# jedisct1/zig-lz4

Hardware: AMD Instinct MI355X
Metric: GiB/s uncompressed, block compress+decompress (higher is better)
Workload: dtype u8

## Files before the change

### zig-lz4_amd/csrc/zlz4_decompress.hip

```cpp
#include <cstdlib>
#include <type_traits>

#include "zlz4_device.hpp"
#include "zlz4_launch.hpp"

#ifdef ZLZ4_STAMPS
__device__ unsigned long long g_zlz4_dstamps[16];
#define DSTAMP_DECL unsigned long long st_acc[16] = {0,0,0,0,0,0,0,0,0,0,0,0,0,0,0,0}; unsigned long long st_last = __builtin_amdgcn_s_memtime();
#define DSTAMP(i) do { unsigned long long st_now; __builtin_amdgcn_sched_barrier(0); \
                      asm volatile("s_memtime %0\n\ts_waitcnt lgkmcnt(0)" : "=s"(st_now) :: "memory"); \
                      __builtin_amdgcn_sched_barrier(0); st_acc[i] += st_now - st_last; st_last = st_now; } while (0)
#define DSTAMP_ADD(i, n) do { st_acc[i] += (n); } while (0)
#define DSTAMP_FLUSH do { if (lane == 0) for (int st_k = 0; st_k < 16; st_k++) atomicAdd(&g_zlz4_dstamps[st_k], st_acc[st_k]); } while (0)
#else
#define DSTAMP_DECL
#define DSTAMP(i)
#define DSTAMP_ADD(i, n)
#define DSTAMP_FLUSH
#endif

namespace zlz4 {

__device__ __forceinline__ uint32_t ld16(const uint8_t *p) { uint16_t v; __builtin_memcpy(&v, p, 2); return v; }
__device__ __forceinline__ uint64_t ld64u(const uint8_t *p) { uint64_t v; __builtin_memcpy(&v, p, 8); return v; }

template <bool kWrite, bool kLaneCopy = false, bool kPhases = kLaneCopy, bool kDict = false, bool kBound = false,
          bool kPartial = false>
__global__ __launch_bounds__(256) __attribute__((amdgpu_waves_per_eu(kDict ? 8 : 1))) void k_decompress_safe(
    const uint8_t *__restrict__ d_in, const uint64_t *__restrict__ d_in_off,
    const uint32_t *__restrict__ d_in_len, uint8_t *d_out, const uint64_t *__restrict__ d_out_off,
    const uint32_t *__restrict__ d_out_cap, int64_t *__restrict__ d_result, uint32_t nblocks, uint32_t min_phase_tokens,
    const uint8_t *__restrict__ d_dict, const uint64_t *__restrict__ d_dict_off, const uint32_t *__restrict__ d_dict_len) {
    constexpr uint32_t short_max = kLaneCopy ? 32u : 0u;
    const uint32_t lane = threadIdx.x & 63u;
    const uint32_t blk = rfl(blockIdx.x * (blockDim.x >> 6) + (threadIdx.x >> 6));
    if (blk >= nblocks) return;

    const uint8_t *src = d_in + d_in_off[blk];
    uint8_t *dst = d_out + d_out_off[blk];
    const uint32_t iend = rfl(d_in_len[blk]);
    const uint32_t oend = rfl(d_out_cap[blk]);
    uint32_t lo = 0;
    if constexpr (kBound) {
        lo = rfl(d_dict_len[nblocks + blk]);
        if (lo >= kBoundInvalid) {
            if (lane == 0 && lo == kBoundInvalid) d_result[blk] = kErrInvalidState;
            return;
        }
    }
    const uint8_t *dend = nullptr, *dbase = nullptr;
    uint32_t dlen = 0;
    if constexpr (kDict) {
        const uint32_t dl = rfl(d_dict_len[blk]);
        dend = d_dict + d_dict_off[blk] + dl;
        dbase = dend - 65536;
        dlen = dl < 65536u ? dl : 65536u;
    }

    int64_t res = 0;
    uint32_t ip = 0, op = 0;

    if (iend != 0 && oend != 0) {
        uint32_t wbase = 0;
        uint32_t w = (lane < iend) ? src[lane] : 0u;
        DSTAMP_DECL
        uint32_t pml = 0, po = 0, pof = 0;
        u32x4 pa = {0, 0, 0, 0}, pb = {0, 0, 0, 0};
        constexpr uint32_t kNone = 0xFFFFFFFFu;
        uint32_t pd0 = 0, pd1 = 0, pdo0 = kNone, pdo1 = kNone;
        auto flush_pending = [&]() {
            if (!kWrite) return;
            if constexpr (kLaneCopy) {
                if (pdo0 != kNone) __builtin_memcpy(dst + pdo0, &pd0, 4);
                if (pdo1 != kNone) __builtin_memcpy(dst + pdo1, &pd1, 4);
                pdo0 = pdo1 = kNone;
            }
            if (pml != 0) {
                if (pml >= 16u) {
                    st128(dst + po, pa);
                    for (uint32_t k = 80u; k + 16u <= pml; k += 16u)
                        st128(dst + (po + k), ld128(kDict && po < pof ? dend - (pof - po) + k : dst + (po - pof + k)));
                    st128(dst + (po + pml - 16u), pb);
                } else if (pml >= 8u) {
                    const uint32_t sh = pml - 8u;
                    const bool hi4 = sh >= 4u;
                    const uint32_t x = hi4 ? pa.y : pa.x, y = hi4 ? pa.z : pa.y, z = hi4 ? pa.w : pa.z;
                    const u32x2 a = {pa.x, pa.y};
                    const u32x2 b = {__builtin_amdgcn_alignbyte(y, x, sh & 3u), __builtin_amdgcn_alignbyte(z, y, sh & 3u)};
                    __builtin_memcpy(dst + po, &a, 8); __builtin_memcpy(dst + (po + sh), &b, 8);
                } else {
                    const uint32_t sh = pml - 4u;
                    const uint32_t a = pa.x, b = __builtin_amdgcn_alignbyte(pa.y, pa.x, sh);
                    __builtin_memcpy(dst + po, &a, 4); __builtin_memcpy(dst + (po + sh), &b, 4);
                }
            }
            pml = 0;
        };
        auto reload = [&](uint32_t pos) {
            wbase = pos;
            w = (pos + lane < iend) ? src[pos + lane] : 0u;
        };
        auto fetch = [&](uint32_t pos) -> uint32_t {
            if (pos - wbase >= 64u) reload(pos);
            return rdlane(w, pos - wbase);
        };

        for (;;) {
            if (ip >= iend) break;
            if constexpr (kPartial) { if (op >= oend) break; }
            DSTAMP(6);
            if ((uint64_t)ip + 68u <= iend) {
              auto woff = [&](uint32_t p) { const uint32_t a = p + lane; return a + 4u <= iend ? a : iend - 4u; };
              auto wload_async = [&](uint32_t p) {
                  uint32_t r;
                  asm volatile("global_load_dword %0, %1, %2" : "=v"(r) : "v"(woff(p)), "s"(src) : "memory");
                  return r;
              };
              uint32_t xbase = ip, tdummy = 0;
              uint32_t X0 = ld32(src + woff(xbase)), X1 = ld32(src + woff(xbase + 64u));
              uint32_t X2 = wload_async(xbase + 128u);
              asm volatile("s_waitcnt vmcnt(0)" : "+v"(X2), "+v"(X0), "+v"(X1));
              for (;;) {
                const uint32_t xi = ip - xbase + lane;
                const uint32_t xa = shfl(X0, xi & 63u), xb = shfl(X1, xi & 63u);
                const uint32_t w4 = xi < 64u ? xa : xb;
                const uint32_t b0 = w4 & 0xFFu, b1 = (w4 >> 8) & 0xFFu;
                uint32_t lit = b0 >> 4, hl = 1u;
                bool cx = false;
                if (lit == 15u) { cx = (b1 == 255u); lit += b1; hl = 2u; }
                const uint32_t mpos = lane + hl + lit;
                const uint32_t mw = shfl(w4, mpos & 63u);
                const uint32_t off = mw & 0xFFFFu;
                uint32_t mlc = b0 & 15u, slen = hl + lit + 2u;
                if (mlc == 15u) { const uint32_t e2 = (mw >> 16) & 0xFFu; cx = cx || (e2 == 255u); mlc += e2; slen += 1u; }
                const uint32_t ml = mlc + kMinMatch;
                const uint32_t nxt = lane + slen;
                const bool ok = !cx && mpos <= 63u && nxt <= 64u && off != 0u;
                const uint32_t ol = lit + ml;
                const uint32_t pkv = ok ? (nxt | (ol << 7)) : 0xFFFFFFFFu;
                DSTAMP(0);
                const uint32_t orem = oend - op;
                const uint32_t room0 = kWrite ? (orem >= 32u ? orem - 32u : 0u) : orem;
                const uint32_t room = rfl(room0 < 4095u ? room0 : 4095u);
                uint32_t pos, T, wa, wpk, wt;
                uint64_t R;
                const uint64_t okm = ballot(ok);
                const uint32_t pk2v = nxt | ((nxt < 64u && ((okm >> (nxt & 63u)) & 1ull)) ? 0x80u : 0u) | (ol << 8);
                if (room0 >= 7100u && (okm & 1ull)) {
                    asm volatile(
                        "s_mov_b64 %[R], 0\n\t"
                        "s_mov_b32 %[T], 0\n\t"
                        "s_mov_b32 %[A], 0\n\t"
                        "s_nop 3\n"
                        "1:\n\t"
                        "v_readlane_b32 %[pk], %[pkv], %[A]\n\t"
                        "s_and_b32 %[B], %[pk], 0x7f\n\t"
                        "s_bitset1_b64 %[R], %[A]\n\t"
                        "s_lshr_b32 %[t], %[pk], 8\n\t"
                        "s_add_u32 %[T], %[T], %[t]\n\t"
                        "s_bitcmp1_b32 %[pk], 7\n\t"
                        "s_cbranch_scc0 4f\n\t"
                        "v_readlane_b32 %[pk], %[pkv], %[B]\n\t"
                        "s_and_b32 %[A], %[pk], 0x7f\n\t"
                        "s_bitset1_b64 %[R], %[B]\n\t"
                        "s_lshr_b32 %[t], %[pk], 8\n\t"
                        "s_add_u32 %[T], %[T], %[t]\n\t"
                        "s_bitcmp1_b32 %[pk], 7\n\t"
                        "s_cbranch_scc1 1b\n\t"
                        "s_mov_b32 %[B], %[A]\n"
                        "4:\n"
                        : [R] "=&s"(R), [T] "=&s"(T), [A] "=&s"(wa), [B] "=&s"(pos), [pk] "=&s"(wpk), [t] "=&s"(wt)
                        : [pkv] "v"(pk2v)
                        : "scc");
                } else
                asm volatile(
                    "s_mov_b64 %[R], 0\n\t"
                    "s_mov_b32 %[T], 0\n\t"
                    "s_mov_b32 %[A], 0\n\t"
                    "s_nop 3\n"
                    "1:\n\t"
                    "v_readlane_b32 %[pk], %[pkv], %[A]\n\t"
                    "s_and_b32 %[B], %[pk], 0x7f\n\t"
                    "s_lshr_b32 %[t], %[pk], 7\n\t"
                    "s_add_u32 %[t], %[t], %[T]\n\t"
                    "s_cmp_gt_u32 %[t], %[room]\n\t"
                    "s_cbranch_scc1 3f\n\t"
                    "s_bitset1_b64 %[R], %[A]\n\t"
                    "s_mov_b32 %[T], %[t]\n\t"
                    "s_cmp_gt_u32 %[B], 63\n\t"
                    "s_cbranch_scc1 4f\n\t"
                    "v_readlane_b32 %[pk], %[pkv], %[B]\n\t"
                    "s_and_b32 %[A], %[pk], 0x7f\n\t"
                    "s_lshr_b32 %[t], %[pk], 7\n\t"
                    "s_add_u32 %[t], %[t], %[T]\n\t"
                    "s_cmp_gt_u32 %[t], %[room]\n\t"
                    "s_cbranch_scc1 4f\n\t"
                    "s_bitset1_b64 %[R], %[B]\n\t"
                    "s_mov_b32 %[T], %[t]\n\t"
                    "s_cmp_lt_u32 %[A], 64\n\t"
                    "s_cbranch_scc1 1b\n"
                    "3:\n\t"
                    "s_mov_b32 %[B], %[A]\n"
                    "4:\n"
                    : [R] "=&s"(R), [T] "=&s"(T), [A] "=&s"(wa), [B] "=&s"(pos), [pk] "=&s"(wpk), [t] "=&s"(wt)
                    : [pkv] "v"(pkv), [room] "s"(room)
                    : "scc");
                DSTAMP(1);
                uint32_t relv = 0;
                const uint64_t R_walk = R;
                const uint32_t T_walk = T, pos_walk = pos;
                bool viol_err = false;
                const uint32_t op0 = op;
                if (R != 0) {
                    const bool real0 = in_mask(R);
                    const uint32_t x = real0 ? ol : 0u;
                    relv = wave_incl_scan(x) - x;
                    const uint32_t lit0 = rdlane(lit, 0);
                    viol_err = off + lo > op0 + relv + lit;
                    if constexpr (kDict) {
                        const uint32_t pr = op0 + relv + lit, need = kLaneCopy ? ml : (ml > 16u ? ml : 16u);
                        viol_err = viol_err && (off - pr < need || off - pr > dlen);
                    }
                    bool viol = viol_err;
                    if (kWrite) viol = viol || (off + lit0 < relv + ol);
                    const uint64_t vm = R & ballot(viol);
                    if (vm != 0) {
                        const uint32_t fb = first_lane(vm);
                        R &= (1ull << fb) - 1ull;
                        T = rdlane(relv, fb);
                        pos = fb;
                    }
                }
                DSTAMP(2);
                asm volatile("s_waitcnt vmcnt(1)" : "+v"(X2), "+v"(pa), "+v"(pb), "+v"(pd0), "+v"(pd1), "+v"(tdummy));
                if (R == 0) break;
                DSTAMP_ADD(8, 1);
                auto cap_short = [&]() {
                    if constexpr (kWrite && kLaneCopy) {
                        if ((uint32_t)__popcll(R) <= 16u) return;
                        const uint64_t S = R & ballot(ml <= short_max);
                        if ((uint32_t)__popcll(S) > 16u) {
                            const uint32_t fb = first_lane(S & ballot(lane_rank(S) == 16u));
                            R &= (1ull << fb) - 1ull;
                            T = rdlane(relv, fb);
                            pos = fb;
                            DSTAMP_ADD(13, 1);
                        }
                    }
                };
                auto copy_side = [&](auto later_phase) {
                if (kWrite) {
                    flush_pending();
                    DSTAMP(7);
                    const uint64_t below = R & (~0ull >> (63u - lane));
                    const uint32_t kl = 63u - (uint32_t)__builtin_clzll(below | 1ull);
                    const uint32_t q = shfl(relv | (lit << 16), kl);
                    const uint32_t qlit = q >> 16;
                    const uint32_t d = lane - kl - (qlit >= 15u ? 2u : 1u);
                    if (d < qlit && (!decltype(later_phase)::value || below != 0)) dst[op0 + (q & 0xFFFFu) + d] = (uint8_t)b0;
                    DSTAMP(3);
                    const uint64_t Sm = R & ballot(ml <= short_max), Lm = R & ~Sm;
                    const uint32_t po_t = op0 + relv + lit;
                    [[maybe_unused]] const bool shortm = in_mask(Sm);
                    const uint64_t H1 = (Lm & ballot(ml > 32u)) << 1, H2 = (Lm & ballot(ml > 64u)) << 2;
                    const uint32_t om = off | (ml << 16);
                    const uint32_t om1 = wave_shr1(om), po1 = wave_shr1(po_t);
                    const uint32_t om2 = wave_shr1(om1), po2 = wave_shr1(po1);
                    if (in_mask(Lm | H1 | H2)) {
                        const bool h1 = in_mask(H1), h2 = in_mask(H2);
                        const uint32_t t_om = h1 ? om1 : (h2 ? om2 : om), t_po = h1 ? po1 : (h2 ? po2 : po_t);
                        const uint32_t t_off = t_om & 0xFFFFu, t_ml = t_om >> 16;
                        const uint32_t pf = h1 ? 16u : (h2 ? 48u : 0u);
                        const uint32_t rest = t_ml - 16u - pf;
                        const uint32_t pl = pf == 0u ? t_ml : (rest < 16u ? 16u : (rest < 32u ? rest : 32u));
                        static_assert(!kLaneCopy || short_max >= 15u, "a lane-copy token lane must hold >= 16 bytes");
                        if constexpr (kDict) {
                            const uint64_t ma = (t_off > t_po ? (uint64_t)(uintptr_t)dbase + (t_po - t_off + 65536u)
                                                              : (uint64_t)(uintptr_t)dst + (t_po - t_off)) + pf;
                            asm volatile("global_load_dwordx4 %0, %1, off" : "+v"(pa) : "v"(ma) : "memory");
                            if (kLaneCopy || pl >= 16u)
                                asm volatile("global_load_dwordx4 %0, %1, off" : "+v"(pb) : "v"(ma + (pl - 16u)) : "memory");
                        } else {
                            const uint32_t mo = t_po - t_off + pf;
                            asm volatile("global_load_dwordx4 %0, %1, %2" : "+v"(pa) : "v"(mo), "s"(dst) : "memory");
                            if (kLaneCopy || pl >= 16u)
                                asm volatile("global_load_dwordx4 %0, %1, %2" : "+v"(pb) : "v"(mo + pl - 16u), "s"(dst) : "memory");
                        }
                        pml = pl; po = t_po + pf; pof = t_off;
                    }
                    if constexpr (kLaneCopy) {
                        const uint32_t ns = (uint32_t)__popcll(Sm);
                        const uint32_t rk = lane_rank(Sm);
                        const uint32_t lead = (lane & ~7u) << 2, k4 = (lane & 7u) * 4u, grp = lane >> 3;
                        auto round = [&](uint32_t g0, uint32_t &pd, uint32_t &pdo) {
                            const uint32_t rel = rk - g0;
                            const uint32_t dest = (shortm && rel < 8u ? rel * 8u : 63u) << 2;
                            const uint32_t s_po = (uint32_t)__builtin_amdgcn_ds_permute((int)dest, (int)po_t);
                            const uint32_t s_om = (uint32_t)__builtin_amdgcn_ds_permute((int)dest, (int)(off | (ml << 16)));
                            const uint32_t g_po = (uint32_t)__builtin_amdgcn_ds_bpermute((int)lead, (int)s_po);
                            const uint32_t g_om = (uint32_t)__builtin_amdgcn_ds_bpermute((int)lead, (int)s_om);
                            const uint32_t g_ml = g_om >> 16, g_mo = g_po - (g_om & 0xFFFFu);
                            const bool act = g0 + grp < ns && k4 < g_ml;
                            const uint32_t pk = k4 + 4u <= g_ml ? k4 : g_ml - 4u;
                            if (act) {
                                if constexpr (kDict) {
                                    const uint64_t ga = g_po < (g_om & 0xFFFFu) ? (uint64_t)(uintptr_t)dbase + (g_mo + pk + 65536u)
                                                                                : (uint64_t)(uintptr_t)dst + (g_mo + pk);
                                    asm volatile("global_load_dword %0, %1, off" : "+v"(pd) : "v"(ga) : "memory");
                                } else
                                    asm volatile("global_load_dword %0, %1, %2" : "+v"(pd) : "v"(g_mo + pk), "s"(dst) : "memory");
                                pdo = g_po + pk;
                            }
                        };
                        round(0u, pd0, pdo0);
                        if (ns > 8u) round(8u, pd1, pdo1);
                    }
                    DSTAMP(4);
                }
                };
                cap_short();
                DSTAMP_ADD(9, __builtin_popcountll(R));
                copy_side(std::false_type{});
                if constexpr (kWrite && kPhases) {
                    for (uint32_t phase = 1; phase < 6u && pos != pos_walk; phase++) {
                        const uint32_t first = pos, tbase = T;
                        const uint64_t Rn = R_walk & ~((1ull << first) - 1ull);
                        if ((uint32_t)__builtin_popcountll(Rn) < min_phase_tokens) break;
                        const uint32_t lit_f = rdlane(lit, first);
                        const bool violn = viol_err || (off + lit_f < (relv - tbase) + ol);
                        const uint64_t vmn = Rn & ballot(violn);
                        if ((vmn >> first) & 1ull) break;
                        if (vmn != 0) {
                            const uint32_t fb = first_lane(vmn);
                            R = Rn & ((1ull << fb) - 1ull);
                            T = rdlane(relv, fb);
                            pos = fb;
                        } else {
                            R = Rn; T = T_walk; pos = pos_walk;
                        }
                        DSTAMP_ADD(12, 1);
                        cap_short();
                        DSTAMP_ADD(9, __builtin_popcountll(R));
                        asm volatile("s_waitcnt vmcnt(0)" : "+v"(pa), "+v"(pb), "+v"(pd0), "+v"(pd1), "+v"(tdummy), "+v"(X2));
                        copy_side(std::true_type{});
#ifdef ZLZ4_STAMPS
                        if (phase == 5u && pos != pos_walk) DSTAMP_ADD(14, 1);
#endif
                    }
                }
                op += T;
                ip += pos;
                if ((uint64_t)ip + 68u > iend) break;
                {
                    const bool adv = ip - xbase >= 64u;
                    X0 = adv ? X1 : X0; X1 = adv ? X2 : X1; xbase += adv ? 64u : 0u;
                    X2 = wload_async(xbase + 128u);
                    const uint32_t ta = xbase + 128u + 1024u;
                    const uint32_t toff = ta < iend ? ta : iend - 1u;
                    asm volatile("global_load_ubyte %0, %1, %2" : "+v"(tdummy) : "v"(toff), "s"(src) : "memory");
                }
              }
              asm volatile("s_waitcnt vmcnt(0)" : "+v"(X2), "+v"(pa), "+v"(pb), "+v"(pd0), "+v"(pd1), "+v"(tdummy));
              if (ip >= iend) { flush_pending(); break; }
            }
            flush_pending();
            DSTAMP_ADD(11, 1);
            if (ip - wbase > 44u) reload(ip);
            {
                const uint32_t i0 = ip - wbase;
                const uint32_t token = rdlane(w, i0);
                const uint32_t lit = token >> 4, mlc = token & 15u;
                const uint32_t in_rem = iend - ip - 1u;
                if (lit != 15u && mlc != 15u && in_rem >= lit + 2u) {
                    if constexpr (kPartial) {
                        if (lit >= oend - op) {
                            if (lane > i0 && lane <= i0 + (oend - op)) dst[op + (lane - i0 - 1u)] = (uint8_t)w;
                            op = oend;
                            break;
                        }
                    } else
                    if (lit > oend - op) { res = kErrOutputTooSmall; break; }
                    if (kWrite && lane > i0 && lane <= i0 + lit) dst[op + (lane - i0 - 1u)] = (uint8_t)w;
                    op += lit;
                    const uint32_t offset = rdlane(w, i0 + 1u + lit) | (rdlane(w, i0 + 2u + lit) << 8);
                    ip += 3u + lit;
                    if (offset == 0) { res = kErrCorrupted; break; }
                    uint32_t ml = mlc + kMinMatch;
                    if constexpr (kPartial) { if (ml > oend - op) ml = oend - op; } else
                    if (ml > oend - op) { res = kErrOutputTooSmall; break; }
                    if (offset > op) {
                        if (!kDict || offset - op > dlen) { res = kErrCorrupted; break; }
                    } else if (kBound && offset + lo > op) { res = kErrCorrupted; break; }
                    if (kWrite) {
                        const uint8_t *m = dst + (op - offset);
                        uint32_t k = lane;
                        if (offset < ml) {
                            if (offset == 1u) k = 0;
                            else { while (k >= offset) k -= offset; }
                        }
                        if constexpr (kDict) {
                            if (lane < ml) dst[op + lane] = op + k < offset ? *(dend - (offset - op - k)) : dst[op + k - offset];
                        } else {
                            if (lane < ml) dst[op + lane] = m[k];
                        }
                    }
                    op += ml;
                    continue;
                }
            }
            const uint32_t token = fetch(ip);
            ip += 1;
            uint32_t lit = token >> 4;
            if (lit == 15u) {
                bool bad = false;
                for (;;) {
                    if (ip >= iend) { bad = true; break; }
                    const uint32_t s = fetch(ip);
                    ip += 1;
                    lit += s;
                    if (lit > 0xFFFF0000u) lit = 0xFFFF0000u;
                    if (s != 255u) break;
                }
                if (bad) { res = kErrCorrupted; break; }
            }
            if (lit > 0) {
                if (lit > iend - ip) { res = kErrCorrupted; break; }
                if constexpr (!kPartial) { if (lit > oend - op) { res = kErrOutputTooSmall; break; } }
                const uint32_t nl = kPartial && lit > oend - op ? oend - op : lit;
                if (!kWrite) {
                } else if (lit <= 64u) {
                    if (ip - wbase + lit > 64u) reload(ip);
                    const uint32_t j0 = ip - wbase;
                    if (lane >= j0 && lane < j0 + nl) dst[op + (lane - j0)] = (uint8_t)w;
                } else {
                    copy_bytes(dst + op, src + ip, nl, lane);
                }
                ip += lit;
                op += nl;
                if constexpr (kPartial) { if (op >= oend) break; }
            }
            if (ip >= iend) break;
            if (iend - ip < 2u) { res = kErrCorrupted; break; }
            const uint32_t offset = fetch(ip) | (fetch(ip + 1u) << 8);
            ip += 2;
            if (offset == 0) { res = kErrCorrupted; break; }
            uint32_t ml = token & 15u;
            if (ml == 15u) {
                bool bad = false;
                for (;;) {
                    if (ip >= iend) { bad = true; break; }
                    const uint32_t s = fetch(ip);
                    ip += 1;
                    ml += s;
                    if (ml > 0xFFFF0000u) ml = 0xFFFF0000u;
                    if (s != 255u) break;
                }
                if (bad) { res = kErrCorrupted; break; }
            }
            ml += kMinMatch;
            if constexpr (kPartial) {
                if (ml > oend - op) ml = oend - op;
            } else if (ml > oend - op) { res = kErrOutputTooSmall; break; }
            if (offset > op) {
                if (!kDict || offset - op > dlen) { res = kErrCorrupted; break; }
            } else if (kBound && offset + lo > op) { res = kErrCorrupted; break; }
            if constexpr (kDict) {
                if (offset > op) {
                    const uint32_t a = offset - op, n1 = a < ml ? a : ml;
                    if (kWrite) copy_bytes(dst + op, dend - a, n1, lane);
                    op += n1;
                    ml -= n1;
                }
            }
            const uint8_t *m = dst + (op - offset);
            uint8_t *o = dst + op;
            if (!kWrite) {
            } else if (offset >= ml || offset >= 1024u) {
                copy_bytes(o, m, ml, lane);
            } else if (offset >= 64u) {
                uint32_t made = 0;
                while (made < ml) {
                    const uint32_t have = made + offset, left = ml - made;
                    const uint32_t n1 = have < left ? have : left;
                    copy_bytes(o + made, m, n1, lane);
                    made += n1;
                }
            } else {
                const uint32_t cs = 64u - (64u % offset);
                const uint8_t v = m[lane % offset];
                if (lane < cs)
                    for (uint32_t k = lane; k < ml; k += cs) o[k] = v;
            }
            op += ml;
        }
        flush_pending();
        if (res == 0) res = (int64_t)op;
        DSTAMP(5);
        DSTAMP_FLUSH;
    }
    if (lane == 0) d_result[blk] = res;
}


__global__ __launch_bounds__(64) void k_decompress_lane(
    const uint8_t *__restrict__ d_in, const uint64_t *__restrict__ d_in_off,
    const uint32_t *__restrict__ d_in_len, uint8_t *d_out, const uint64_t *__restrict__ d_out_off,
    const uint32_t *__restrict__ d_out_cap, int64_t *__restrict__ d_result, uint32_t nblocks) {
  for (uint32_t blk = blockIdx.x * blockDim.x + threadIdx.x; blk < nblocks; blk += gridDim.x * blockDim.x) {
    const uint8_t *src = d_in + d_in_off[blk];
    uint8_t *dst = d_out + d_out_off[blk];
    const uint32_t iend = d_in_len[blk], oend = d_out_cap[blk];
    int64_t res = 0;
    uint32_t ip = 0, op = 0;
    if (iend != 0 && oend != 0) {
        u32x4 w = {0, 0, 0, 0};
        bool have_w = false;
        if (16u <= iend) { w = ld128(src); have_w = true; }
        for (;;) {
            if (ip >= iend) break;
            if (have_w) {
                const uint32_t tok = w.x & 0xFFu;
                const uint32_t lit = tok >> 4, mlc = tok & 15u;
                if (lit <= 13u && mlc != 15u && (uint64_t)op + lit + 48u <= oend) {
                    const uint32_t oi = 1u + lit;
                    const uint32_t d0 = oi >> 2, sh = (oi & 3u) * 8u;
                    const uint32_t lo = d0 == 0 ? w.x : (d0 == 1 ? w.y : (d0 == 2 ? w.z : w.w));
                    const uint32_t hi = d0 == 0 ? w.y : (d0 == 1 ? w.z : w.w);
                    const uint32_t offset = (uint32_t)((((uint64_t)hi << 32) | lo) >> sh) & 0xFFFFu;
                    const uint32_t nip = ip + 3u + lit;
                    u32x4 wn = {0, 0, 0, 0};
                    const bool have_n = (uint64_t)nip + 16u <= iend;
                    if (have_n) wn = ld128(src + nip);
                    u32x4 ls;
                    ls.x = (w.x >> 8) | (w.y << 24); ls.y = (w.y >> 8) | (w.z << 24);
                    ls.z = (w.z >> 8) | (w.w << 24); ls.w = w.w >> 8;
                    st128(dst + op, ls);
                    op += lit;
                    ip = nip;
                    if (offset == 0) { res = kErrCorrupted; break; }
                    const uint32_t ml = mlc + kMinMatch;
                    if (offset > op) { res = kErrCorrupted; break; }
                    const uint8_t *m = dst + (op - offset);
                    uint8_t *o = dst + op;
                    if (offset >= 16u) {
                        st128(o, ld128(m));
                        if (ml > 16u) st128(o + 16u, ld128(m + 16u));
                    } else if (offset >= 8u) {
                        for (uint32_t k = 0; k < ml; k += 8u) { const uint64_t v = ld64u(m + k); __builtin_memcpy(o + k, &v, 8); }
                    } else {
                        for (uint32_t k = 0; k < ml; k++) o[k] = m[k];
                    }
                    op += ml;
                    w = wn;
                    have_w = have_n;
                    continue;
                }
            }
            const uint32_t token = src[ip];
            ip += 1;
            uint32_t lit = token >> 4;
            if (lit == 15u) {
                bool bad = false;
                for (;;) {
                    if (ip >= iend) { bad = true; break; }
                    const uint32_t s = src[ip];
                    ip += 1;
                    lit += s;
                    if (lit > 0xFFFF0000u) lit = 0xFFFF0000u;
                    if (s != 255u) break;
                }
                if (bad) { res = kErrCorrupted; break; }
            }
            if (lit > 0) {
                if (lit > iend - ip) { res = kErrCorrupted; break; }
                if (lit > oend - op) { res = kErrOutputTooSmall; break; }
                uint32_t k = 0;
                while (k < lit && (uint64_t)ip + k + 16u <= iend && (uint64_t)op + k + 16u <= oend) {
                    st128(dst + op + k, ld128(src + ip + k));
                    k += 16u;
                }
                for (; k < lit; k++) dst[op + k] = src[ip + k];
                ip += lit;
                op += lit;
            }
            if (ip >= iend) break;
            if (iend - ip < 2u) { res = kErrCorrupted; break; }
            const uint32_t offset = ld16(src + ip);
            ip += 2;
            if (offset == 0) { res = kErrCorrupted; break; }
            uint32_t ml = token & 15u;
            if (ml == 15u) {
                bool bad = false;
                for (;;) {
                    if (ip >= iend) { bad = true; break; }
                    const uint32_t s = src[ip];
                    ip += 1;
                    ml += s;
                    if (ml > 0xFFFF0000u) ml = 0xFFFF0000u;
                    if (s != 255u) break;
                }
                if (bad) { res = kErrCorrupted; break; }
            }
            ml += kMinMatch;
            if (ml > oend - op) { res = kErrOutputTooSmall; break; }
            if (offset > op) { res = kErrCorrupted; break; }
            const uint8_t *m = dst + (op - offset);
            uint8_t *o = dst + op;
            uint32_t k = 0;
            if (offset >= 16u) {
                while (k < ml && (uint64_t)op + k + 16u <= oend) { st128(o + k, ld128(m + k)); k += 16u; }
            } else if (offset >= 8u) {
                while (k < ml && (uint64_t)op + k + 8u <= oend) { const uint64_t v = ld64u(m + k); __builtin_memcpy(o + k, &v, 8); k += 8u; }
            }
            for (; k < ml; k++) o[k] = m[k];
            op += ml;
            have_w = (uint64_t)ip + 16u <= iend;
            if (have_w) w = ld128(src + ip);
        }
        if (res == 0) res = (int64_t)op;
    }
    d_result[blk] = res;
  }
}

}

namespace {

constexpr uint32_t kLaneCopyMinBlocks = 6144;

long long tune_int(const char *name, long long dflt) { const char *e = zlz4_tune_env(name); return e ? atoll(e) : dflt; }

struct SafeArgs {
    const uint8_t *d_in; const uint64_t *d_in_off; const uint32_t *d_in_len;
    uint8_t *d_out; const uint64_t *d_out_off; const uint32_t *d_out_cap;
    int64_t *d_result; uint32_t nblocks;
    const uint8_t *d_dict; const uint64_t *d_dict_off; const uint32_t *d_dict_len;
};

struct SafeShape {
    uint32_t grid, threads, lds, min_phase_tokens;
    bool lane_copy;
};
SafeShape safe_shape(uint32_t nblocks, bool knobs, uint32_t min_phase_tokens = 3u) {
    static const uint32_t wpw_env = [] { const uint32_t v = (uint32_t)tune_int("ZLZ4_DECOMP_WPW", 4);
                                         return (v == 1u || v == 2u || v == 4u) ? v : 4u; }();
    static const uint32_t phase_min_env = (uint32_t)tune_int("ZLZ4_DECOMP_PHASE_MIN", 3);
    const uint32_t waves_per_wg = knobs ? wpw_env : 4u;
    return {grid_of(nblocks, waves_per_wg), 64u * waves_per_wg, 0u, knobs ? phase_min_env : min_phase_tokens,
            nblocks >= kLaneCopyMinBlocks};
}

template <bool kWrite, bool kLaneCopy, bool kPhases = kLaneCopy, bool kDict = false, bool kBound = false,
          bool kPartial = false>
int launch_safe(hipStream_t stream, const SafeShape &sh, const SafeArgs &a) {
    hipLaunchKernelGGL((zlz4::k_decompress_safe<kWrite, kLaneCopy, kPhases, kDict, kBound, kPartial>), dim3(sh.grid), dim3(sh.threads),
                       sh.lds, stream, a.d_in, a.d_in_off, a.d_in_len, a.d_out, a.d_out_off, a.d_out_cap, a.d_result, a.nblocks,
                       sh.min_phase_tokens, a.d_dict, a.d_dict_off, a.d_dict_len);
    return zlz4_launch_status();
}

}

extern "C" int zlz4_launch_decompress_safe(hipStream_t stream, const uint8_t *d_in, const uint64_t *d_in_off,
                                           const uint32_t *d_in_len, uint8_t *d_out, const uint64_t *d_out_off,
                                           const uint32_t *d_out_cap, int64_t *d_result, uint32_t nblocks) {
    if (nblocks == 0) return 0;
    static const uint32_t lane_min = (uint32_t)tune_int("ZLZ4_DECOMP_LANE_MIN", 0xFFFFFFFFll);
    if (nblocks >= lane_min) {
        static const uint32_t lanes_env = (uint32_t)tune_int("ZLZ4_DECOMP_LANES", 0);
        uint32_t lanes = nblocks >= 524288u ? 64u : (nblocks >= 262144u ? 32u : 16u);
        if (lanes_env >= 1 && lanes_env <= 64) lanes = lanes_env;
        static const uint32_t max_lanes = (uint32_t)tune_int("ZLZ4_DECOMP_MAXLANES", 0);
        uint32_t grid = (nblocks + lanes - 1u) / lanes;
        if (max_lanes && (uint64_t)grid * lanes > max_lanes) grid = (max_lanes + lanes - 1u) / lanes;
        hipLaunchKernelGGL(zlz4::k_decompress_lane, dim3(grid), dim3(lanes), 0, stream, d_in, d_in_off,
                           d_in_len, d_out, d_out_off, d_out_cap, d_result, nblocks);
        return zlz4_launch_status();
    }
    SafeShape sh = safe_shape(nblocks, true);
    static const uint32_t dyn_lds = (uint32_t)tune_int("ZLZ4_DECOMP_LDS", 0);
    static const int short_env = (int)tune_int("ZLZ4_DECOMP_SHORT", -1);
    static const bool no_phases = tune_int("ZLZ4_DECOMP_PHASES", 1) == 0;
    sh.lds = dyn_lds;
    if (short_env >= 0) sh.lane_copy = short_env != 0;
    const SafeArgs a = {d_in, d_in_off, d_in_len, d_out, d_out_off, d_out_cap, d_result, nblocks, nullptr, nullptr, nullptr};
    if (sh.lane_copy && no_phases) return launch_safe<true, true, false>(stream, sh, a);
    return sh.lane_copy ? launch_safe<true, true>(stream, sh, a) : launch_safe<true, false>(stream, sh, a);
}

extern "C" int zlz4_launch_decompress_safe_using_dict(hipStream_t stream, const uint8_t *d_in, const uint64_t *d_in_off,
                                                      const uint32_t *d_in_len, uint8_t *d_out, const uint64_t *d_out_off,
                                                      const uint32_t *d_out_cap, int64_t *d_result, uint32_t nblocks,
                                                      const uint8_t *d_dict, const uint64_t *d_dict_off,
                                                      const uint32_t *d_dict_len) {
    if (nblocks == 0) return 0;
    const SafeShape sh = safe_shape(nblocks, true);
    const SafeArgs a = {d_in, d_in_off, d_in_len, d_out, d_out_off, d_out_cap, d_result, nblocks, d_dict, d_dict_off, d_dict_len};
    return sh.lane_copy ? launch_safe<true, true, true, true>(stream, sh, a) : launch_safe<true, false, false, true>(stream, sh, a);
}

extern "C" int zlz4_launch_decompress_safe_prefix(hipStream_t stream, const uint8_t *d_in, const uint64_t *d_in_off,
                                                  const uint32_t *d_in_len, uint8_t *d_out, const uint64_t *d_out_off,
                                                  const uint32_t *d_out_cap, int64_t *d_result, uint32_t nblocks) {
    if (nblocks == 0) return 0;
    const SafeShape sh = safe_shape(nblocks, false);
    const SafeArgs a = {d_in, d_in_off, d_in_len, d_out, d_out_off, d_out_cap, d_result, nblocks, nullptr, nullptr, nullptr};
    return sh.lane_copy ? launch_safe<true, true, true, false, false, true>(stream, sh, a)
                        : launch_safe<true, false, false, false, false, true>(stream, sh, a);
}

extern "C" int zlz4_launch_decompress_safe_prefix_using_dict(hipStream_t stream, const uint8_t *d_in, const uint64_t *d_in_off,
                                                             const uint32_t *d_in_len, uint8_t *d_out,
                                                             const uint64_t *d_out_off, const uint32_t *d_out_cap,
                                                             int64_t *d_result, uint32_t nblocks, const uint8_t *d_dict,
                                                             const uint64_t *d_dict_off, const uint32_t *d_dict_len) {
    if (nblocks == 0) return 0;
    const SafeShape sh = safe_shape(nblocks, false);
    const SafeArgs a = {d_in, d_in_off, d_in_len, d_out, d_out_off, d_out_cap, d_result, nblocks, d_dict, d_dict_off, d_dict_len};
    return sh.lane_copy ? launch_safe<true, true, true, true, false, true>(stream, sh, a)
                        : launch_safe<true, false, false, true, false, true>(stream, sh, a);
}

extern "C" int zlz4_launch_decompress_safe_bound(hipStream_t stream, const uint8_t *d_in, const uint64_t *d_in_off,
                                                 const uint32_t *d_in_len, uint8_t *d_out, const uint64_t *d_out_off,
                                                 const uint32_t *d_out_cap, int64_t *d_result, uint32_t nblocks,
                                                 const uint8_t *d_dict, const uint64_t *d_dict_off,
                                                 const uint32_t *d_dict_len, int with_dict) {
    if (nblocks == 0) return 0;
    const SafeShape sh = safe_shape(nblocks, false);
    const SafeArgs a = {d_in, d_in_off, d_in_len, d_out, d_out_off, d_out_cap, d_result, nblocks, d_dict, d_dict_off, d_dict_len};
    if (with_dict)
        return sh.lane_copy ? launch_safe<true, true, true, true, true>(stream, sh, a)
                            : launch_safe<true, false, false, true, true>(stream, sh, a);
    return sh.lane_copy ? launch_safe<true, true, true, false, true>(stream, sh, a)
                        : launch_safe<true, false, false, false, true>(stream, sh, a);
}

extern "C" int zlz4_launch_decompress_sizes(hipStream_t stream, const uint8_t *d_in, const uint64_t *d_in_off,
                                            const uint32_t *d_in_len, const uint64_t *d_out_off,
                                            const uint32_t *d_out_cap, int64_t *d_result, uint32_t nblocks) {
    if (nblocks == 0) return 0;
    const SafeArgs a = {d_in, d_in_off, d_in_len, nullptr, d_out_off, d_out_cap, d_result, nblocks, nullptr, nullptr, nullptr};
    return launch_safe<false, false>(stream, safe_shape(nblocks, false, 0u), a);
}

extern "C" int zlz4_launch_decompress_sizes_using_dict(hipStream_t stream, const uint8_t *d_in, const uint64_t *d_in_off,
                                                       const uint32_t *d_in_len, const uint64_t *d_out_off,
                                                       const uint32_t *d_out_cap, int64_t *d_result, uint32_t nblocks,
                                                       const uint64_t *d_dict_off, const uint32_t *d_dict_len) {
    if (nblocks == 0) return 0;
    const SafeArgs a = {d_in, d_in_off, d_in_len, nullptr, d_out_off, d_out_cap, d_result, nblocks, nullptr, d_dict_off, d_dict_len};
    return launch_safe<false, false, false, true>(stream, safe_shape(nblocks, false, 0u), a);
}

#ifdef ZLZ4_STAMPS
extern "C" int zlz4_debug_read_dstamps(unsigned long long *out16, int reset) {
    if (hipMemcpyFromSymbol(out16, HIP_SYMBOL(g_zlz4_dstamps), 16 * sizeof(unsigned long long)) != hipSuccess) return ZLZ4_ERR_DEVICE;
    if (reset) {
        unsigned long long z[16] = {0};
        if (hipMemcpyToSymbol(HIP_SYMBOL(g_zlz4_dstamps), z, sizeof z) != hipSuccess) return ZLZ4_ERR_DEVICE;
    }
    return 0;
}
#endif
```

### zig-lz4_amd/csrc/zlz4_device.hpp

```cpp
#pragma once
#include <hip/hip_runtime.h>
#include <stdint.h>
#include <stdlib.h>

#ifdef ZLZ4_TUNING
static inline const char *zlz4_tune_env(const char *name) { return getenv(name); }
#else
static inline const char *zlz4_tune_env(const char *) { return nullptr; }
#endif

namespace zlz4 {

typedef uint32_t u32x4 __attribute__((ext_vector_type(4)));
typedef uint32_t u32x2 __attribute__((ext_vector_type(2)));

constexpr uint32_t kMinMatch = 4;
constexpr uint32_t kLastLiterals = 5;
constexpr uint32_t kMfLimit = 12;
constexpr uint32_t kMaxInput = 0x7E000000u;
constexpr uint32_t kMaxDist = 65535u;
constexpr uint32_t kHashMul = 2654435761u;

constexpr int64_t kErrOutputTooSmall = -1;
constexpr int64_t kErrInputTooLarge = -2;
constexpr int64_t kErrCorrupted = -3;
constexpr int64_t kErrInvalidState = -5;

constexpr uint32_t kBoundSkip = 0xFFFFFFFFu, kBoundInvalid = 0xFFFFFFFEu, kBoundMax = 0xFFFF0000u;

__device__ __forceinline__ uint32_t rfl(uint32_t v) { return __builtin_amdgcn_readfirstlane(v); }
__device__ __forceinline__ uint32_t rdlane(uint32_t v, uint32_t l) { return __builtin_amdgcn_readlane(v, l); }
__device__ __forceinline__ uint64_t ballot(bool p) { return __ballot(p); }
__device__ __forceinline__ uint32_t first_lane(uint64_t m) { return (uint32_t)__ffsll((long long)m) - 1u; }
__device__ __forceinline__ uint32_t shfl(uint32_t v, uint32_t src_lane) {
    return (uint32_t)__builtin_amdgcn_ds_bpermute((int)(src_lane << 2), (int)v);
}

__device__ __forceinline__ uint32_t lane_rank(uint64_t mask) {
    return __builtin_amdgcn_mbcnt_hi((uint32_t)(mask >> 32), __builtin_amdgcn_mbcnt_lo((uint32_t)mask, 0u));
}
__device__ __forceinline__ bool in_mask(uint64_t mask) { return __builtin_amdgcn_inverse_ballot_w64(mask); }

__device__ __forceinline__ uint32_t wave_shr1(uint32_t v) {
    return (uint32_t)__builtin_amdgcn_update_dpp(0, (int)v, 0x138, 0xF, 0xF, true);
}

template <uint32_t kOff>
__device__ __forceinline__ uint32_t add_wrap_byte(uint32_t a) {
    static_assert(kOff <= 64u, "inline constant");
    uint32_t r;
    asm("v_add_u32_sdwa %0, %1, %2 dst_sel:BYTE_0 dst_unused:UNUSED_PAD src0_sel:DWORD src1_sel:DWORD"
        : "=v"(r) : "v"(a), "n"(kOff));
    return r;
}

__device__ __forceinline__ uint32_t wrlane(uint32_t val, uint32_t l, uint32_t old) {
    return (__lane_id() == l) ? val : old;
}

__device__ __forceinline__ uint32_t ld32(const uint8_t *p) { uint32_t v; __builtin_memcpy(&v, p, 4); return v; }
__device__ __forceinline__ u32x4 ld128(const uint8_t *p) { u32x4 v; __builtin_memcpy(&v, p, 16); return v; }
__device__ __forceinline__ void st128(uint8_t *p, u32x4 v) { __builtin_memcpy(p, &v, 16); }

__device__ __forceinline__ uint32_t first_diff16(u32x4 a, u32x4 b) {
    const uint32_t x0 = a.x ^ b.x, x1 = a.y ^ b.y, x2 = a.z ^ b.z, x3 = a.w ^ b.w;
    if (x0) return (uint32_t)__builtin_ctz(x0) >> 3;
    if (x1) return 4u + ((uint32_t)__builtin_ctz(x1) >> 3);
    if (x2) return 8u + ((uint32_t)__builtin_ctz(x2) >> 3);
    if (x3) return 12u + ((uint32_t)__builtin_ctz(x3) >> 3);
    return 16u;
}

__device__ __forceinline__ uint32_t first_diff16_sel(u32x4 a, u32x4 b) {
    const uint32_t x0 = a.x ^ b.x, x1 = a.y ^ b.y, x2 = a.z ^ b.z, x3 = a.w ^ b.w;
    const uint32_t lo = x0 ? x0 : x1, hi = x2 ? x2 : x3;
    const uint32_t blo = x0 ? 0u : 4u, bhi = x2 ? 8u : 12u;
    const bool in_lo = (x0 | x1) != 0;
    const uint32_t x = in_lo ? lo : hi;
    const uint32_t base = in_lo ? blo : bhi;
    return x ? base + ((uint32_t)__builtin_ctz(x) >> 3) : 16u;
}

__device__ __forceinline__ void copy_bytes(uint8_t *dst, const uint8_t *src, uint32_t n, uint32_t lane) {
    uint32_t k = lane * 16u;
    for (; k + 16u <= n; k += 1024u) st128(dst + k, ld128(src + k));
    const uint32_t t0 = n & ~15u;
    if (t0 + lane < n && lane < 16u) dst[t0 + lane] = src[t0 + lane];
}

__device__ __forceinline__ uint32_t wave_incl_scan(uint32_t x) {
    x += (uint32_t)__builtin_amdgcn_update_dpp(0, (int)x, 0x111, 0xF, 0xF, true);
    x += (uint32_t)__builtin_amdgcn_update_dpp(0, (int)x, 0x112, 0xF, 0xF, true);
    x += (uint32_t)__builtin_amdgcn_update_dpp(0, (int)x, 0x114, 0xF, 0xF, true);
    x += (uint32_t)__builtin_amdgcn_update_dpp(0, (int)x, 0x118, 0xF, 0xF, true);
    x += (uint32_t)__builtin_amdgcn_update_dpp(0, (int)x, 0x142, 0xA, 0xF, false);
    x += (uint32_t)__builtin_amdgcn_update_dpp(0, (int)x, 0x143, 0xC, 0xF, false);
    return x;
}

__device__ __forceinline__ uint64_t rfl64(uint64_t v) { return ((uint64_t)rfl((uint32_t)(v >> 32)) << 32) | rfl((uint32_t)v); }
__device__ __forceinline__ uint32_t byte_at(const uint8_t *p) { return rfl((uint32_t)*p); }

template <bool kWrite, bool kDict = false, bool kBound = false, bool kPartial = false>
__device__ int64_t decode_block_wave(const uint8_t *src, uint32_t iend, uint8_t *out, uint32_t oend, uint32_t hist,
                                     uint32_t lane, const uint8_t *tend = nullptr, uint32_t inframe = 0, uint32_t lo = 0) {
    if (iend == 0 || oend == 0) return 0;
    uint32_t ip = 0, op = 0;
    for (;;) {
        if (ip >= iend) break;
        if constexpr (kPartial) { if (op >= oend) break; }
        const uint32_t token = byte_at(src + ip++);
        uint32_t lit = token >> 4;
        if (lit == 15u) {
            for (;;) {
                if (ip >= iend) return kErrCorrupted;
                const uint32_t b = byte_at(src + ip++);
                lit += b;
                if (lit > 0xFFFF0000u) lit = 0xFFFF0000u;
                if (b != 255u) break;
            }
        }
        if (lit > 0) {
            if (lit > iend - ip) return kErrCorrupted;
            if constexpr (kPartial) {
                const uint32_t nl = lit < oend - op ? lit : oend - op;
                if (kWrite) copy_bytes(out + op, src + ip, nl, lane);
                ip += lit; op += nl;
                if (op >= oend) break;
            } else {
                if (lit > oend - op) return kErrOutputTooSmall;
                if (kWrite) copy_bytes(out + op, src + ip, lit, lane);
                ip += lit; op += lit;
            }
        }
        if (ip >= iend) break;
        if (iend - ip < 2u) return kErrCorrupted;
        const uint32_t offset = byte_at(src + ip) | (byte_at(src + ip + 1) << 8);
        ip += 2;
        if (offset == 0) return kErrCorrupted;
        uint32_t ml = token & 15u;
        if (ml == 15u) {
            for (;;) {
                if (ip >= iend) return kErrCorrupted;
                const uint32_t b = byte_at(src + ip++);
                ml += b;
                if (ml > 0xFFFF0000u) ml = 0xFFFF0000u;
                if (b != 255u) break;
            }
        }
        ml += kMinMatch;
        if constexpr (kPartial) {
            if (ml > oend - op) ml = oend - op;
        } else {
            if (ml > oend - op) return kErrOutputTooSmall;
        }
        if (offset > op && offset - op > hist) return kErrCorrupted;
        if constexpr (kBound) {
            if (offset + lo > op) return kErrCorrupted;
        }
        if (kWrite) {
            uint8_t *o = out + op;
            uint32_t n = ml;
            if constexpr (kDict) {
                if (offset > op + inframe) {
                    const uint32_t a = offset - op - inframe, n1 = a < n ? a : n;
                    copy_bytes(o, tend - a, n1, lane);
                    o += n1;
                    n -= n1;
                }
            }
            const uint8_t *m = o - offset;
            if (n == 0) {
            } else if (offset >= n || offset >= 1024u) {
                copy_bytes(o, m, n, lane);
            } else {
                uint32_t made = 0;
                while (made < n) {
                    const uint32_t have = made + offset, left = n - made;
                    const uint32_t n1 = have < left ? have : left;
                    copy_bytes(o + made, m, n1, lane);
                    made += n1;
                }
            }
        }
        op += ml;
    }
    return (int64_t)op;
}

__device__ __forceinline__ uint32_t ext_len_bytes(uint32_t v) { return v >= 15u ? 1u + (v - 15u) / 255u : 0u; }

__device__ __forceinline__ void write_ext_len(uint8_t *p, uint32_t v, uint32_t lane) {
    const uint32_t rem = v - 15u;
    const uint32_t n255 = rem / 255u;
    for (uint32_t k = lane; k < n255; k += 64u) p[k] = 255;
    if (lane == 0) p[n255] = (uint8_t)(rem - n255 * 255u);
}

}
```

Measured before the change: 88.70.

## Replace serial scalar token-chain walk with parallel pointer-jumping orbit in decompress

In write mode, the serial scalar readlane loop that follows the chain of token start positions across the 64-byte window is replaced. Reachable token lanes are now found in parallel with ds_permute/ds_bpermute pointer doubling (token_orbit). The room limit is then applied afterwards through a prefix scan plus ballot rather than being checked inside the loop. The goal is to shorten the latency of serially chained v_readlane/s_cbranch steps per window, at the cost of several LDS permute rounds and extra ballots. It also forces the 16-byte store path for pending matches when lane-copy mode is on, and adds a tuning env switch for choosing the walk.

Result: no change. 89.51, median of 6 (+0.9%).

```diff
diff --git a/zig-lz4_amd/csrc/zlz4_decompress.hip b/zig-lz4_amd/csrc/zlz4_decompress.hip
--- a/zig-lz4_amd/csrc/zlz4_decompress.hip
+++ b/zig-lz4_amd/csrc/zlz4_decompress.hip
@@ -25,7 +25,7 @@
 __device__ __forceinline__ uint64_t ld64u(const uint8_t *p) { uint64_t v; __builtin_memcpy(&v, p, 8); return v; }
 
 template <bool kWrite, bool kLaneCopy = false, bool kPhases = kLaneCopy, bool kDict = false, bool kBound = false,
-          bool kPartial = false>
+          bool kPartial = false, bool kOrbit = kWrite>
 __global__ __launch_bounds__(256) __attribute__((amdgpu_waves_per_eu(kDict ? 8 : 1))) void k_decompress_safe(
     const uint8_t *__restrict__ d_in, const uint64_t *__restrict__ d_in_off,
     const uint32_t *__restrict__ d_in_len, uint8_t *d_out, const uint64_t *__restrict__ d_out_off,
@@ -76,7 +76,7 @@
                 pdo0 = pdo1 = kNone;
             }
             if (pml != 0) {
-                if (pml >= 16u) {
+                if (kLaneCopy || pml >= 16u) {
                     st128(dst + po, pa);
                     for (uint32_t k = 80u; k + 16u <= pml; k += 16u)
                         st128(dst + (po + k), ld128(kDict && po < pof ? dend - (pof - po) + k : dst + (po - pof + k)));
@@ -135,18 +135,51 @@
                 if (mlc == 15u) { const uint32_t e2 = (mw >> 16) & 0xFFu; cx = cx || (e2 == 255u); mlc += e2; slen += 1u; }
                 const uint32_t ml = mlc + kMinMatch;
                 const uint32_t nxt = lane + slen;
-                const bool ok = !cx && mpos <= 63u && nxt <= 64u && off != 0u;
                 const uint32_t ol = lit + ml;
-                const uint32_t pkv = ok ? (nxt | (ol << 7)) : 0xFFFFFFFFu;
                 DSTAMP(0);
                 const uint32_t orem = oend - op;
                 const uint32_t room0 = kWrite ? (orem >= 32u ? orem - 32u : 0u) : orem;
-                const uint32_t room = rfl(room0 < 4095u ? room0 : 4095u);
-                uint32_t pos, T, wa, wpk, wt;
+                uint32_t pos = 0, T = 0;
                 uint64_t R;
-                const uint64_t okm = ballot(ok);
-                const uint32_t pk2v = nxt | ((nxt < 64u && ((okm >> (nxt & 63u)) & 1ull)) ? 0x80u : 0u) | (ol << 8);
-                if (room0 >= 7100u && (okm & 1ull)) {
+                if constexpr (kOrbit) {
+                    const uint64_t cxm = (ballot(b0 >> 4 == 15u) & ballot(b1 == 255u)) |
+                                         (ballot((b0 & 15u) == 15u) & ballot(((mw >> 16) & 0xFFu) == 255u));
+                    const uint64_t okm = ballot(nxt <= 64u) & ballot(off != 0u) & ~cxm;
+                    R = token_orbit(nxt, okm);
+                } else {
+                    const bool ok = !cx && mpos <= 63u && nxt <= 64u && off != 0u;
+                    const uint32_t pkv = ok ? (nxt | (ol << 7)) : 0xFFFFFFFFu;
+                    const uint32_t room = rfl(room0 < 4095u ? room0 : 4095u);
+                    uint32_t wa, wpk, wt;
+                    const uint64_t okm = ballot(ok);
+                    const uint32_t pk2v = nxt | ((nxt < 64u && ((okm >> (nxt & 63u)) & 1ull)) ? 0x80u : 0u) | (ol << 8);
+                    if (room0 >= 7100u && (okm & 1ull)) {
+                        asm volatile(
+                            "s_mov_b64 %[R], 0\n\t"
+                            "s_mov_b32 %[T], 0\n\t"
+                            "s_mov_b32 %[A], 0\n\t"
+                            "s_nop 3\n"
+                            "1:\n\t"
+                            "v_readlane_b32 %[pk], %[pkv], %[A]\n\t"
+                            "s_and_b32 %[B], %[pk], 0x7f\n\t"
+                            "s_bitset1_b64 %[R], %[A]\n\t"
+                            "s_lshr_b32 %[t], %[pk], 8\n\t"
+                            "s_add_u32 %[T], %[T], %[t]\n\t"
+                            "s_bitcmp1_b32 %[pk], 7\n\t"
+                            "s_cbranch_scc0 4f\n\t"
+                            "v_readlane_b32 %[pk], %[pkv], %[B]\n\t"
+                            "s_and_b32 %[A], %[pk], 0x7f\n\t"
+                            "s_bitset1_b64 %[R], %[B]\n\t"
+                            "s_lshr_b32 %[t], %[pk], 8\n\t"
+                            "s_add_u32 %[T], %[T], %[t]\n\t"
+                            "s_bitcmp1_b32 %[pk], 7\n\t"
+                            "s_cbranch_scc1 1b\n\t"
+                            "s_mov_b32 %[B], %[A]\n"
+                            "4:\n"
+                            : [R] "=&s"(R), [T] "=&s"(T), [A] "=&s"(wa), [B] "=&s"(pos), [pk] "=&s"(wpk), [t] "=&s"(wt)
+                            : [pkv] "v"(pk2v)
+                            : "scc");
+                    } else
                     asm volatile(
                         "s_mov_b64 %[R], 0\n\t"
                         "s_mov_b32 %[T], 0\n\t"
@@ -155,66 +188,55 @@
                         "1:\n\t"
                         "v_readlane_b32 %[pk], %[pkv], %[A]\n\t"
                         "s_and_b32 %[B], %[pk], 0x7f\n\t"
+                        "s_lshr_b32 %[t], %[pk], 7\n\t"
+                        "s_add_u32 %[t], %[t], %[T]\n\t"
+                        "s_cmp_gt_u32 %[t], %[room]\n\t"
+                        "s_cbranch_scc1 3f\n\t"
                         "s_bitset1_b64 %[R], %[A]\n\t"
-                        "s_lshr_b32 %[t], %[pk], 8\n\t"
-                        "s_add_u32 %[T], %[T], %[t]\n\t"
-                        "s_bitcmp1_b32 %[pk], 7\n\t"
-                        "s_cbranch_scc0 4f\n\t"
+                        "s_mov_b32 %[T], %[t]\n\t"
+                        "s_cmp_gt_u32 %[B], 63\n\t"
+                        "s_cbranch_scc1 4f\n\t"
                         "v_readlane_b32 %[pk], %[pkv], %[B]\n\t"
                         "s_and_b32 %[A], %[pk], 0x7f\n\t"
+                        "s_lshr_b32 %[t], %[pk], 7\n\t"
+                        "s_add_u32 %[t], %[t], %[T]\n\t"
+                        "s_cmp_gt_u32 %[t], %[room]\n\t"
+                        "s_cbranch_scc1 4f\n\t"
                         "s_bitset1_b64 %[R], %[B]\n\t"
-                        "s_lshr_b32 %[t], %[pk], 8\n\t"
-                        "s_add_u32 %[T], %[T], %[t]\n\t"
-                        "s_bitcmp1_b32 %[pk], 7\n\t"
-                        "s_cbranch_scc1 1b\n\t"
+                        "s_mov_b32 %[T], %[t]\n\t"
+                        "s_cmp_lt_u32 %[A], 64\n\t"
+                        "s_cbranch_scc1 1b\n"
+                        "3:\n\t"
                         "s_mov_b32 %[B], %[A]\n"
                         "4:\n"
                         : [R] "=&s"(R), [T] "=&s"(T), [A] "=&s"(wa), [B] "=&s"(pos), [pk] "=&s"(wpk), [t] "=&s"(wt)
-                        : [pkv] "v"(pk2v)
+                        : [pkv] "v"(pkv), [room] "s"(room)
                         : "scc");
-                } else
-                asm volatile(
-                    "s_mov_b64 %[R], 0\n\t"
-                    "s_mov_b32 %[T], 0\n\t"
-                    "s_mov_b32 %[A], 0\n\t"
-                    "s_nop 3\n"
-                    "1:\n\t"
-                    "v_readlane_b32 %[pk], %[pkv], %[A]\n\t"
-                    "s_and_b32 %[B], %[pk], 0x7f\n\t"
-                    "s_lshr_b32 %[t], %[pk], 7\n\t"
-                    "s_add_u32 %[t], %[t], %[T]\n\t"
-                    "s_cmp_gt_u32 %[t], %[room]\n\t"
-                    "s_cbranch_scc1 3f\n\t"
-                    "s_bitset1_b64 %[R], %[A]\n\t"
-                    "s_mov_b32 %[T], %[t]\n\t"
-                    "s_cmp_gt_u32 %[B], 63\n\t"
-                    "s_cbranch_scc1 4f\n\t"
-                    "v_readlane_b32 %[pk], %[pkv], %[B]\n\t"
-                    "s_and_b32 %[A], %[pk], 0x7f\n\t"
-                    "s_lshr_b32 %[t], %[pk], 7\n\t"
-                    "s_add_u32 %[t], %[t], %[T]\n\t"
-                    "s_cmp_gt_u32 %[t], %[room]\n\t"
-                    "s_cbranch_scc1 4f\n\t"
-                    "s_bitset1_b64 %[R], %[B]\n\t"
-                    "s_mov_b32 %[T], %[t]\n\t"
-                    "s_cmp_lt_u32 %[A], 64\n\t"
-                    "s_cbranch_scc1 1b\n"
-                    "3:\n\t"
-                    "s_mov_b32 %[B], %[A]\n"
-                    "4:\n"
-                    : [R] "=&s"(R), [T] "=&s"(T), [A] "=&s"(wa), [B] "=&s"(pos), [pk] "=&s"(wpk), [t] "=&s"(wt)
-                    : [pkv] "v"(pkv), [room] "s"(room)
-                    : "scc");
+                }
                 DSTAMP(1);
                 uint32_t relv = 0;
-                const uint64_t R_walk = R;
-                const uint32_t T_walk = T, pos_walk = pos;
+                uint64_t R_walk = R;
+                uint32_t T_walk = T, pos_walk = pos;
                 bool viol_err = false;
                 const uint32_t op0 = op;
                 if (R != 0) {
                     const bool real0 = in_mask(R);
                     const uint32_t x = real0 ? ol : 0u;
                     relv = wave_incl_scan(x) - x;
+                    if constexpr (kOrbit) {
+                        const uint32_t room = room0 >= 7100u ? 0xFFFFFFFFu : (room0 < 4095u ? room0 : 4095u);
+                        const uint32_t last = 63u - (uint32_t)__builtin_clzll(R), tend = relv + ol;
+                        pos = rdlane(nxt, last);
+                        T = rdlane(tend, last);
+                        const uint64_t rm = R & ballot(tend > room);
+                        if (rm != 0) {
+                            const uint32_t fb = first_lane(rm);
+                            R &= (1ull << fb) - 1ull;
+                            T = rdlane(relv, fb);
+                            pos = fb;
+                        }
+                        R_walk = R; T_walk = T; pos_walk = pos;
+                    }
                     const uint32_t lit0 = rdlane(lit, 0);
                     viol_err = off + lo > op0 + relv + lit;
                     if constexpr (kDict) {
@@ -654,10 +676,18 @@
 template <bool kWrite, bool kLaneCopy, bool kPhases = kLaneCopy, bool kDict = false, bool kBound = false,
           bool kPartial = false>
 int launch_safe(hipStream_t stream, const SafeShape &sh, const SafeArgs &a) {
-    hipLaunchKernelGGL((zlz4::k_decompress_safe<kWrite, kLaneCopy, kPhases, kDict, kBound, kPartial>), dim3(sh.grid), dim3(sh.threads),
-                       sh.lds, stream, a.d_in, a.d_in_off, a.d_in_len, a.d_out, a.d_out_off, a.d_out_cap, a.d_result, a.nblocks,
-                       sh.min_phase_tokens, a.d_dict, a.d_dict_off, a.d_dict_len);
-    return zlz4_launch_status();
+    auto go = [&](auto orbit) {
+        hipLaunchKernelGGL((zlz4::k_decompress_safe<kWrite, kLaneCopy, kPhases, kDict, kBound, kPartial, decltype(orbit)::value>),
+                           dim3(sh.grid), dim3(sh.threads), sh.lds, stream, a.d_in, a.d_in_off, a.d_in_len, a.d_out, a.d_out_off,
+                           a.d_out_cap, a.d_result, a.nblocks, sh.min_phase_tokens, a.d_dict, a.d_dict_off, a.d_dict_len);
+        return zlz4_launch_status();
+    };
+#ifdef ZLZ4_TUNING
+    static const int walk_env = (int)tune_int("ZLZ4_DECOMP_WALK", -1);
+    if (walk_env == 0) return go(std::false_type{});
+    if (walk_env == 1) return go(std::true_type{});
+#endif
+    return go(std::integral_constant<bool, kWrite>{});
 }
 
 }
diff --git a/zig-lz4_amd/csrc/zlz4_device.hpp b/zig-lz4_amd/csrc/zlz4_device.hpp
--- a/zig-lz4_amd/csrc/zlz4_device.hpp
+++ b/zig-lz4_amd/csrc/zlz4_device.hpp
@@ -43,6 +43,18 @@
 
 __device__ __forceinline__ uint32_t wave_shr1(uint32_t v) {
     return (uint32_t)__builtin_amdgcn_update_dpp(0, (int)v, 0x138, 0xF, 0xF, true);
+}
+
+__device__ __forceinline__ uint64_t token_orbit(uint32_t nxt, uint64_t okm) {
+    uint32_t d4 = in_mask(okm & ballot(nxt < 64u)) ? nxt << 2 : 252u;
+    uint32_t out = __lane_id() == 0u ? 0u : 252u;
+#pragma unroll
+    for (uint32_t r = 0; r < 5u; r++) {
+        const uint32_t got = (uint32_t)__builtin_amdgcn_ds_permute((int)(d4 | out), -1);
+        if (r < 4u) d4 = (uint32_t)__builtin_amdgcn_ds_bpermute((int)d4, (int)d4);
+        out &= ~got;
+    }
+    return ballot(out == 0u) & okm;
 }
 
 template <uint32_t kOff>
```
